# Ecogenomics/CheckM

Hardware: NVIDIA B200
Metric: genomes/hour (higher is better)
Workload: dtype int16 (SSV) / u8 (MSV) / int16 (Viterbi) / f32 (Forward, domain definition)

## Files before the change

### checkm_b200/csrc/device_utils.cuh

```cuda
#pragma once
#include <cuda_runtime.h>
#include <cstdint>

namespace ckm {

__device__ __forceinline__ uint32_t smem_u32(const void *p) { return (uint32_t)__cvta_generic_to_shared(p); }

__device__ __forceinline__ uint4 lds128(uint32_t addr) {
  uint4 v;
  asm volatile("ld.shared.v4.u32 {%0,%1,%2,%3}, [%4];" : "=r"(v.x), "=r"(v.y), "=r"(v.z), "=r"(v.w) : "r"(addr));
  return v;
}

__device__ __forceinline__ uint32_t prmt_b32(uint32_t a, uint32_t b, uint32_t c) {
  uint32_t d;
  asm("prmt.b32 %0, %1, %2, %3;" : "=r"(d) : "r"(a), "r"(b), "r"(c));
  return d;
}

__device__ __forceinline__ void mbar_init(uint64_t *bar, int count) {
  asm volatile("mbarrier.init.shared::cta.b64 [%0], %1;" ::"r"(smem_u32(bar)), "r"(count) : "memory");
}
__device__ __forceinline__ void fence_mbar_init() { asm volatile("fence.mbarrier_init.release.cluster;" ::: "memory"); }
__device__ __forceinline__ void fence_proxy_async() { asm volatile("fence.proxy.async.shared::cta;" ::: "memory"); }
__device__ __forceinline__ void mbar_expect_tx(uint64_t *bar, uint32_t bytes) {
  asm volatile("mbarrier.arrive.expect_tx.shared::cta.b64 _, [%0], %1;" ::"r"(smem_u32(bar)), "r"(bytes) : "memory");
}
__device__ __forceinline__ void bulk_g2s(uint32_t dst_smem, const void *src, uint32_t bytes, uint64_t *bar) {
  asm volatile("cp.async.bulk.shared::cluster.global.mbarrier::complete_tx::bytes [%0], [%1], %2, [%3];" ::"r"(dst_smem),
               "l"(src), "r"(bytes), "r"(smem_u32(bar))
               : "memory");
}
__device__ __forceinline__ void mbar_wait(uint64_t *bar, uint32_t parity) {
  asm volatile(
      "{\n"
      ".reg .pred p;\n"
      "WAIT_LOOP:\n"
      "mbarrier.try_wait.parity.shared::cta.b64 p, [%0], %1;\n"
      "@p bra WAIT_DONE;\n"
      "bra WAIT_LOOP;\n"
      "WAIT_DONE:\n"
      "}\n" ::"r"(smem_u32(bar)),
      "r"(parity)
      : "memory");
}

__device__ __forceinline__ int warp_max_int(int v) {
#pragma unroll
  for (int o = 16; o > 0; o >>= 1) v = max(v, __shfl_xor_sync(0xffffffffu, v, o));
  return v;
}
__device__ __forceinline__ float warp_sum_float(float v) {
#pragma unroll
  for (int o = 16; o > 0; o >>= 1) v += __shfl_xor_sync(0xffffffffu, v, o);
  return v;
}
__device__ __forceinline__ unsigned long long warp_sum_ull(unsigned long long v) {
#pragma unroll
  for (int o = 16; o > 0; o >>= 1) v += __shfl_xor_sync(0xffffffffu, v, o);
  return v;
}

__device__ __forceinline__ void atomicOr_u8(uint8_t *base, int64_t idx, unsigned bits) {
  unsigned *w = reinterpret_cast<unsigned *>(base + (idx & ~(int64_t)3));
  atomicOr(w, bits << (8 * (idx & 3)));
}

__device__ __forceinline__ double gumbel_surv(double x, double mu, double lambda) {
  const double y = lambda * (x - mu);
  const double ey = -exp(-y);
  if (fabs(ey) < 5e-9) return -ey;
  return 1.0 - exp(ey);
}
__device__ __forceinline__ double exp_surv(double x, double mu, double lambda) { return (x < mu) ? 1.0 : exp(-lambda * (x - mu)); }
__device__ __forceinline__ double exp_logsurv(double x, double mu, double lambda) { return (x < mu) ? 0.0 : -lambda * (x - mu); }

}
```

### checkm_b200/csrc/engine.hpp

```cpp
#pragma once
#include <cuda_runtime.h>
#include <cstdint>
#include <string>
#include <vector>
#include "../../include/ckm.h"
#include "hmm_model.hpp"

namespace ckm {
constexpr int MAX_MODEL_M = 4608;

constexpr int SSV_I8_WORDS = 8;
__host__ __device__ constexpr int ssv_row_bytes(int J) { return (J == 32) ? 128 * J - 16 * 32 * (SSV_I8_WORDS / 4 - 1) : 128 * J; }
__host__ __device__ constexpr int ssv_table_bytes(int J) { return KPAD * ssv_row_bytes(J); }
__host__ __device__ constexpr int ssv_block_bytes(int J) { return ssv_table_bytes(J) + 768; }
struct TileModel {
  int32_t model;
  int32_t slot0, nslots;
  int32_t chunk;
};

struct TileDesc {
  int32_t J;
  int32_t first_model;
  int32_t nmodels;
  int32_t chain_next;
  int32_t chain_prev;
  int32_t pad;
  int64_t table_off;
};

struct TileGroup {
  int32_t J;
  int32_t first_tile, ntiles;
  int32_t nchains;
  int32_t first_chain;
  int32_t pad;
  int64_t table_off;
  int64_t table_bytes;
};

struct ModelScalars {
  int32_t M;
  int32_t off_cells;
  int32_t Mpad;
  uint8_t tbm_b, tec_b, base_b, bias_b;
  int16_t base_w, xw_e_loop, xw_e_move;
  int16_t msv2_ok;
// ... 21 lines not shown
  EnvScratch, Envs1, EnvOrder1, Envs2, EnvOrder2,
  EnsRegions, EnsMultiIdx, EnsScratchOff, EnsScratch, EnsEnvs, EnsCount, EnsCaps, EnsEnvOff, EnsNeed,
  NtBytes, NtRows, NtPieces, NtStats, NtContigScaf, NtContigLen, NtCounters,
  Gather,
  Count
};

}

struct ckm_models {
  std::vector<ckm::Model> models;
  ckm::ModelScalars *d_scalars = nullptr;
  uint8_t  *d_rbv = nullptr;
  int16_t  *d_rwv = nullptr;
  int16_t  *d_twv = nullptr;
  float    *d_rfv = nullptr;
  float    *d_tfv = nullptr;
  float    *d_bias_eo = nullptr;
  uint4    *d_twb = nullptr;
  uint32_t *d_rmb = nullptr;
  uint32_t *d_rwb = nullptr;
  uint4    *d_twp = nullptr;
  uint32_t *d_rwp = nullptr;
  float4   *d_tfb = nullptr;
  float    *d_rfb = nullptr;
  int64_t   total_cols = 0;
  int       maxM = 0;
  std::vector<ckm::TileDesc>  tiles;
  std::vector<ckm::TileModel> tile_models;
  std::vector<ckm::TileGroup> groups;
  std::vector<int32_t>        chain_first_tile;
  std::vector<int32_t>        chain_ntiles;
  std::vector<int32_t>        ssv_bypass;
  int32_t        *d_ssv_bypass = nullptr;
  ckm::TileDesc  *d_tiles = nullptr;
  ckm::TileModel *d_tile_models = nullptr;
  ckm::TileGroup *d_groups = nullptr;
  int32_t        *d_chain_first_tile = nullptr, *d_chain_ntiles = nullptr;
  uint8_t        *d_tile_blob = nullptr;
  float          *d_tile_A = nullptr;
  int32_t        *d_tile_F = nullptr;
  int32_t        *d_tile_slot_model = nullptr;
  int64_t         tile_blob_bytes = 0;
  ckm_engine     *engine = nullptr;
};

struct ckm_seqdb {
  int32_t nseq = 0, nbins = 0;
  int64_t nres = 0;
  int64_t padded_bytes = 0;
  int32_t maxL = 0;
  std::vector<int64_t> offsets;
  std::vector<int32_t> bin_of_seq, bin_first_seq, bin_nseq;
  std::vector<int32_t> len;
  uint8_t *d_res = nullptr;
  int64_t *d_off = nullptr;
  int32_t *d_len = nullptr;
  int32_t *d_bin = nullptr;
  float   *d_nullsc = nullptr;
  int32_t *d_tjb = nullptr;
  float   *d_msvB = nullptr;
  float   *d_lenA = nullptr, *d_lenB = nullptr;
  int16_t *d_tmove_w = nullptr;
  int32_t *d_order = nullptr;
  int32_t *d_bin_nseq = nullptr;
  ckm_engine *engine = nullptr;
// ... 22 lines not shown
```

### checkm_b200/csrc/kernels_msv.cu

```cuda
#include <algorithm>
#include "engine.hpp"
#include "device_utils.cuh"
#include "stages.hpp"

namespace ckm {


template <int J> __host__ __device__ constexpr int tile_table_bytes() { return ssv_table_bytes(J); }
template <int J> __host__ __device__ constexpr int tile_block_bytes() { return ssv_block_bytes(J); }


template <int J>
__device__ __forceinline__ void ssv_rows(const uint8_t *__restrict__ res, int L, uint32_t tile_smem, int lane, uint32_t sel,
                                         const int16_t *bnd_in, int16_t *bnd_out, uint32_t (&u)[J], uint32_t &xE) {
  constexpr int G = J / 4;
  const uint4 *rp = reinterpret_cast<const uint4 *>(res);
  const uint32_t lane_off = tile_smem + lane * 16;
  constexpr bool I8 = (J == 32);
  constexpr int G0 = I8 ? SSV_I8_WORDS / 4 : 0;
  auto do_row = [&](uint32_t x, int i) {
    const uint32_t row = lane_off + x * ssv_row_bytes(J);
    uint4 e[G];
    if (I8) {
      const uint4 c = lds128(row);
      const uint32_t cw[4] = {c.x, c.y, c.z, c.w};
#pragma unroll
      for (int q = 0; q < SSV_I8_WORDS; ++q) (&e[q >> 2].x)[q & 3] = prmt_b32(cw[q >> 1], 0u, (q & 1) ? 0xB3A2u : 0x9180u);
    }
#pragma unroll
    for (int g = G0; g < G; ++g) e[g] = lds128(row + (g - (I8 ? G0 - 1 : 0)) * 512);
    uint32_t bndw = 0;
    if (bnd_in != nullptr) bndw = (i > 0) ? (uint32_t)(uint16_t)bnd_in[i - 1] : 0u;
    const uint32_t sh = __shfl_sync(0xffffffffu, u[J - 1], (lane + 31) & 31);
#pragma unroll
    for (int q = J - 1; q >= 1; --q) {
      const uint32_t d = (&e[q >> 2].x)[q & 3];
      u[q] = __viaddmax_s16x2_relu(u[q - 1], d, 0x80008000u);
    }
    const uint32_t p0 = __byte_perm(sh, bndw, sel);
    u[0] = __viaddmax_s16x2_relu(p0, e[0].x, 0x80008000u);
#pragma unroll
    for (int q = 0; q < J; q += 2) xE = __vimax3_s16x2(xE, u[q], u[q + 1]);
    if (bnd_out != nullptr && lane == 31) bnd_out[i] = (int16_t)(u[J - 1] >> 16);
  };
  const int nfull = L >> 4;
  uint4 cur = __ldg(rp);
  for (int b = 0; b < nfull; ++b) {
    const uint4 nxt = __ldg(rp + b + 1);
    const uint32_t w4[4] = {cur.x, cur.y, cur.z, cur.w};
#pragma unroll
    for (int r = 0; r < 16; ++r) do_row((w4[r >> 2] >> (8 * (r & 3))) & 0xffu, b * 16 + r);
    cur = nxt;
  }
  const int ntail = ((L & 15) + 3) >> 2;
  for (int t = 0; t < ntail; ++t) {
    const uint32_t w = (t == 0) ? cur.x : (t == 1) ? cur.y : (t == 2) ? cur.z : cur.w;
#pragma unroll
    for (int r = 0; r < 4; ++r) do_row((w >> (8 * r)) & 0xffu, nfull * 16 + t * 4 + r);
  }
}

template <int J>
__global__ void __launch_bounds__(SSV_WARPS * 32, 1) ssv_kernel(SsvParams p) {
  extern __shared__ __align__(128) uint8_t smem[];
  __shared__ __align__(8) uint64_t bar;
  __shared__ int s_unit, s_item;
  __shared__ int16_t su[SSV_WARPS][64];
  const int tid = threadIdx.x, lane = tid & 31, warp = tid >> 5;
  const uint32_t smem_base = smem_u32(smem);
  const uint32_t sel = (lane == 0) ? 0x1054u : 0x3210u;
  constexpr int TB = tile_block_bytes<J>();
  constexpr int I8CAP = (J == 32) ? 127 : 32767;
  if (tid == 0) { mbar_init(&bar, 1); fence_mbar_init(); }
  __syncthreads();
  uint32_t phase = 0;
  int cur_group = -1;
  unsigned long long my_cells = 0;
  int16_t *bndA = p.bnd ? p.bnd + ((int64_t)(blockIdx.x * SSV_WARPS + warp) * 2) * p.bnd_stride : nullptr;
  int16_t *bndB = p.bnd ? bndA + p.bnd_stride : nullptr;

  while (true) {
    __syncthreads();
    if (tid == 0) { s_unit = atomicAdd(p.unit_counter, 1); s_item = 0; }
    __syncthreads();
    const int unit = s_unit;
    if (unit >= p.ngroups * p.nchunks) break;
    const int gi = unit / p.nchunks, chunk = unit % p.nchunks;
    const TileGroup grp = p.groups[p.group_list[gi]];
    if (gi != cur_group) {
      cur_group = gi;
      if (tid == 0) {
        fence_proxy_async();
        mbar_expect_tx(&bar, (uint32_t)grp.table_bytes);
        for (int t = 0; t < grp.ntiles; ++t)
          bulk_g2s(smem_base + t * TB, p.tile_blob + grp.table_off + (int64_t)t * TB, TB, &bar);
      }
      mbar_wait(&bar, phase);
      phase ^= 1;
    }
    const int s_begin = chunk * p.seq_chunk;
    const int s_count = min(p.seq_chunk, p.nseq - s_begin);
    const int nitems = s_count * grp.nchains;
    while (true) {
      int it = 0;
      if (lane == 0) it = atomicAdd(&s_item, 1);
      it = __shfl_sync(0xffffffffu, it, 0);
      if (it >= nitems) break;
      const int s = p.order[s_begin + it / grp.nchains];
      const int chain = grp.first_chain + it % grp.nchains;
      const int L = p.len[s];
      if (L == 0) continue;
      const int t0 = p.chain_first_tile[chain], nt = p.chain_ntiles[chain];
      const int sbin = p.bin[s];
      if (p.tile_active != nullptr && !p.tile_active[(int64_t)sbin * p.ntiles + t0]) continue;
      const uint8_t *res = p.res + p.off[s];
      const float Bs = p.msvB[s];
      const int tjb = p.tjb[s];
      bool chain_cand = false;
      for (int tt = 0; tt < nt; ++tt) {
        const int t = t0 + tt;
        const int tl = t - grp.first_tile;
        const uint32_t tsm = smem_base + tl * TB;
        uint32_t u[J];
#pragma unroll
        for (int q = 0; q < J; ++q) u[q] = 0u;
        uint32_t xE = 0u;
        const int16_t *bin_ = (nt > 1 && tt > 0) ? ((tt & 1) ? bndA : bndB) : nullptr;
        int16_t *bout = (nt > 1 && tt + 1 < nt) ? ((tt & 1) ? bndB : bndA) : nullptr;
        ssv_rows<J>(res, L, tsm, lane, sel, bin_, bout, u, xE);
        my_cells += (unsigned long long)L * (2 * J);
        const uint8_t *meta = smem + tl * TB + tile_table_bytes<J>();
        const float *A = reinterpret_cast<const float *>(meta);
        const int32_t *F = reinterpret_cast<const int32_t *>(meta + 256);
        const int32_t *SM = reinterpret_cast<const int32_t *>(meta + 512);
        const int ulo = (int)(int16_t)(xE & 0xffffu), uhi = (int)(int16_t)(xE >> 16);
        const int thr_lo = min(min((int)floorf(A[lane] + Bs) - 1, F[lane] + tjb), I8CAP);
        const int thr_hi = min(min((int)floorf(A[32 + lane] + Bs) - 1, F[32 + lane] + tjb), I8CAP);
        const bool c_lo = (SM[lane] >= 0) && (ulo >= thr_lo);
        const bool c_hi = (SM[32 + lane] >= 0) && (uhi >= thr_hi);
        const unsigned m_lo = __ballot_sync(0xffffffffu, c_lo), m_hi = __ballot_sync(0xffffffffu, c_hi);
        if ((m_lo | m_hi) == 0u) continue;
        if (nt > 1) { chain_cand = true; continue; }
        su[warp][lane] = (int16_t)ulo; su[warp][32 + lane] = (int16_t)uhi;
        __syncwarp();
        const TileDesc td = p.tiles[t];
        if (lane < td.nmodels) {
          const TileModel tm = p.tile_models[td.first_model + lane];
          const unsigned long long mask = ((unsigned long long)m_hi << 32) | m_lo;
          const unsigned long long range = ((tm.nslots >= 64) ? ~0ull : ((1ull << tm.nslots) - 1ull)) << tm.slot0;
          bool act = (mask & range) != 0ull;
          if (act && p.model_active != nullptr) act = p.model_active[(int64_t)sbin * p.nmodels + tm.model] != 0;
          if (act) {
            int umax = 0;
            for (int z = tm.slot0; z < tm.slot0 + tm.nslots; ++z) umax = max(umax, (int)su[warp][z]);
            const int jbound = min(F[tm.slot0] + tjb, I8CAP);
            if (!p.resolve || umax >= jbound || umax < 1) {
              const int pos = atomicAdd(p.cand_count, 1);
              if (pos < p.cand_cap) p.cand[pos] = make_int2(s, tm.model);
            } else {
              const ModelScalars ms = p.ms[tm.model];
              const int tjbm = min(tjb + (int)ms.tbm_b, 255);
              const int xB0 = max((int)ms.base_b - tjbm, 0);
              const int xJ = max(umax + xB0 - (int)ms.tec_b, 0);
              float usc = ((float)(xJ - tjb) - (float)ms.base_b);
              usc = __fdiv_rn(usc, ms.scale_b);
              usc = __fsub_rn(usc, 3.0f);
              if (p.xj_dense != nullptr) p.xj_dense[(int64_t)p.model_slot[tm.model] * p.nseq + s] = xJ;
              const float nullsc = p.nullsc[s];
              const float seq_score = __fdiv_rn(__fsub_rn(usc, nullsc), 0.69314718055994529f);
              const double P = gumbel_surv((double)seq_score, (double)ms.evparam[0], (double)ms.evparam[1]);
              atomicAdd(p.resolved_count, 1);
              if (P <= p.F1) {
                const int pos = atomicAdd(p.pass_count, 1);
                if (pos < p.pass_cap) {
                  Candidate cd;
                  cd.seq = s; cd.model = tm.model; cd.usc = usc; cd.filtersc = nullsc; cd.vitsc = 0.f; cd.fwdsc = 0.f; cd.P = P;
                  p.pass[pos] = cd;
                }
              }
            }
          }
        }
        __syncwarp();
      }
      if (nt > 1 && chain_cand && lane == 0) {
        const TileModel tm = p.tile_models[p.tiles[t0].first_model];
        bool act = true;
        if (p.model_active != nullptr) act = p.model_active[(int64_t)sbin * p.nmodels + tm.model] != 0;
        if (act) {
          const int pos = atomicAdd(p.cand_count, 1);
          if (pos < p.cand_cap) p.cand[pos] = make_int2(s, tm.model);
        }
      }
    }
  }
  my_cells = warp_sum_ull(my_cells);
  if (lane == 0 && p.cells != nullptr) atomicAdd(p.cells, my_cells);
}

template __global__ void ssv_kernel<4>(SsvParams);
template __global__ void ssv_kernel<8>(SsvParams);
template __global__ void ssv_kernel<16>(SsvParams);
template __global__ void ssv_kernel<32>(SsvParams);

int launch_ssv(int J, const SsvParams &p, int grid, size_t smem_bytes, cudaStream_t stream) {
  cudaError_t e;
  switch (J) {
    case 4:
      e = cudaFuncSetAttribute(ssv_kernel<4>, cudaFuncAttributeMaxDynamicSharedMemorySize, (int)smem_bytes);
      if (e != cudaSuccess) return cuda_fail(e, "cudaFuncSetAttribute(ssv<4>)");
      ssv_kernel<4><<<grid, SSV_WARPS * 32, smem_bytes, stream>>>(p);
      break;
    case 8:
      e = cudaFuncSetAttribute(ssv_kernel<8>, cudaFuncAttributeMaxDynamicSharedMemorySize, (int)smem_bytes);
      if (e != cudaSuccess) return cuda_fail(e, "cudaFuncSetAttribute(ssv<8>)");
      ssv_kernel<8><<<grid, SSV_WARPS * 32, smem_bytes, stream>>>(p);
      break;
    case 16:
      e = cudaFuncSetAttribute(ssv_kernel<16>, cudaFuncAttributeMaxDynamicSharedMemorySize, (int)smem_bytes);
      if (e != cudaSuccess) return cuda_fail(e, "cudaFuncSetAttribute(ssv<16>)");
      ssv_kernel<16><<<grid, SSV_WARPS * 32, smem_bytes, stream>>>(p);
      break;
    case 32:
      e = cudaFuncSetAttribute(ssv_kernel<32>, cudaFuncAttributeMaxDynamicSharedMemorySize, (int)smem_bytes);
      if (e != cudaSuccess) return cuda_fail(e, "cudaFuncSetAttribute(ssv<32>)");
      ssv_kernel<32><<<grid, SSV_WARPS * 32, smem_bytes, stream>>>(p);
      break;
    default: set_error("unsupported tile width"); return CKM_EINVAL;
  }
  e = cudaGetLastError();
  if (e != cudaSuccess) return cuda_fail(e, "ssv_kernel launch");
  return CKM_OK;
}



__global__ void __launch_bounds__(MSV_WARPS * 32) msv_exact_kernel(MsvParams p) {
  extern __shared__ __align__(128) uint8_t smem[];
  const int lane = threadIdx.x & 31, warp = threadIdx.x >> 5;
  uint8_t *row0 = smem + (size_t)warp * 2 * p.row_bytes, *row1 = row0 + p.row_bytes;
  const int ncand = min(*p.cand_count, p.cand_cap);
  for (int c = blockIdx.x * MSV_WARPS + warp; c < ncand; c += gridDim.x * MSV_WARPS) {
    const int2 pr = p.cand[c];
    const int s = pr.x, m = pr.y;
    const ModelScalars ms = p.ms[m];
    if (p.use_blk && ms.msv2_ok) continue;
    const int M = ms.M, L = p.len[s];
    const uint8_t *res = p.res + p.off[s];
    const uint8_t *rbv = p.rbv + (int64_t)ms.off_cells * KPAD;
    const int tjb = p.tjb[s];
    const int tjbm = min(tjb + (int)ms.tbm_b, 255);
    const int bias = ms.bias_b, base = ms.base_b, tec = ms.tec_b;
    for (int k = lane; k <= M + 1; k += 32) { row0[k] = 0; row1[k] = 0; }
    __syncwarp();
    int xJ = 0, xB = max(base - tjbm, 0);
    bool overflow = false;
    uint8_t *prev = row0, *cur = row1;
    for (int i = 0; i < L; ++i) {
      const int x = res[i];
      const uint8_t *rsc = rbv + (int64_t)x * ms.Mpad;
      int xE = 0;
      for (int k = lane + 1; k <= M; k += 32) {
        int sv = max((int)prev[k - 1], xB);
        sv = min(sv + bias, 255);
        sv = max(sv - (int)rsc[k], 0);
// ... 235 lines not shown
```

### checkm_b200/csrc/models.cu

```cuda
#include <algorithm>
#include <cmath>
#include <cstdlib>
#include <cstring>
#include <fstream>
#include <stdexcept>
#include "engine.hpp"

namespace ckm {

static thread_local std::string g_error;
void set_error(const std::string &msg) { g_error = msg; }
const std::string &get_error() { return g_error; }
int cuda_fail(cudaError_t e, const char *what) {
  set_error(std::string("CUDA error: ") + cudaGetErrorString(e) + " in " + what);
  return CKM_ECUDA;
}

static const double kLog2 = 0.69314718055994529;

template <class T>
static int upload(T **dptr, const std::vector<T> &h) {
  size_t bytes = std::max<size_t>(h.size() * sizeof(T), 16);
  CKM_CUDA(cudaMalloc((void **)dptr, bytes));
  if (!h.empty()) CKM_CUDA(cudaMemcpy(*dptr, h.data(), h.size() * sizeof(T), cudaMemcpyHostToDevice));
  return CKM_OK;
}

static int tile_block_bytes_host(int J) { return ssv_block_bytes(J); }

static void build_tiles(ckm_models &db, std::vector<uint8_t> &blob) {
  const int n = (int)db.models.size();
  struct Item { int model, M; };
  const char *pol = std::getenv("CKM_SSV_J");
  int fixedJ = 32;
  if (pol != nullptr) { if (!std::strcmp(pol, "auto")) fixedJ = 0; else fixedJ = std::atoi(pol); }
  if (fixedJ != 0 && fixedJ != 4 && fixedJ != 8 && fixedJ != 16 && fixedJ != 32) fixedJ = 32;
  std::vector<Item> cls[3], longm;
  int Js[3] = {4, 8, 16};
  int chainJ = 16;
  if (fixedJ != 0) { Js[0] = Js[1] = Js[2] = fixedJ; chainJ = (fixedJ == 32) ? 16 : fixedJ; }
  for (int i = 0; i < n; ++i) {
    int M = db.models[i].M;
    if (fixedJ != 0) { if (M <= 64 * fixedJ - 1) cls[0].push_back({i, M}); else longm.push_back({i, M}); }
    else if (M <= 255) cls[0].push_back({i, M});
    else if (M <= 511) cls[1].push_back({i, M});
    else if (M <= 1023) cls[2].push_back({i, M});
    else longm.push_back({i, M});
  }
  struct HostTile { int J; std::vector<TileModel> tm; int used; int chain_prev, chain_next; };
  std::vector<HostTile> tiles;
  std::vector<std::pair<int, int>> chains;
  std::vector<int> tile_class;
  for (int c = 0; c < 3; ++c) {
    auto &v = cls[c];
    std::stable_sort(v.begin(), v.end(), [](const Item &a, const Item &b) { return a.M > b.M; });
    const int J = Js[c];
    size_t first = tiles.size();
    for (const Item &it : v) {
      int W = it.M / J + 1;
      size_t t;
      for (t = first; t < tiles.size(); ++t)
        if (tiles[t].used + W <= 64 && (int)tiles[t].tm.size() < 32) break;
      if (t == tiles.size()) { tiles.push_back({J, {}, 0, 0, 0}); tile_class.push_back(c); }
      tiles[t].tm.push_back({it.model, tiles[t].used, W, 0});
      tiles[t].used += W;
    }
    for (size_t t = first; t < tiles.size(); ++t) chains.push_back({(int)t, 1});
  }
  const int chunk_cells = 64 * chainJ;
  const int64_t cap = 200000;
  db.ssv_bypass.clear();
  for (const Item &it : longm) {
    int ncells = it.M + 1;
    int nch = (ncells + chunk_cells - 1) / chunk_cells;
    if ((int64_t)nch * tile_block_bytes_host(chainJ) > cap) { db.ssv_bypass.push_back(it.model); continue; }
    chains.push_back({(int)tiles.size(), nch});
    for (int c = 0; c < nch; ++c) {
      HostTile ht{chainJ, {}, 64, c > 0, c + 1 < nch};
      ht.tm.push_back({it.model, 0, 64, c});
      tiles.push_back(ht);
      tile_class.push_back(3);
    }
  }
  db.tiles.clear(); db.tile_models.clear(); db.groups.clear(); db.chain_first_tile.clear(); db.chain_ntiles.clear();
  int64_t off = 0;
  for (size_t t = 0; t < tiles.size(); ++t) {
    TileDesc td{};
    td.J = tiles[t].J; td.first_model = (int)db.tile_models.size(); td.nmodels = (int)tiles[t].tm.size();
    td.chain_next = tiles[t].chain_next; td.chain_prev = tiles[t].chain_prev; td.table_off = off;
    for (auto &tm : tiles[t].tm) db.tile_models.push_back(tm);
    db.tiles.push_back(td);
    off += tile_block_bytes_host(td.J);
  }
  blob.assign((size_t)off, 0);
  {
    TileGroup g{}; bool open = false; int64_t gbytes = 0;
    for (size_t c = 0; c < chains.size(); ++c) {
      int t0 = chains[c].first, nt = chains[c].second, J = tiles[t0].J;
      int64_t need = (int64_t)nt * tile_block_bytes_host(J);
      if (need > cap) throw std::runtime_error("model " + db.models[tiles[t0].tm[0].model].name + " is too long for the SSV tiles");
      if (open && (g.J != J || gbytes + need > cap)) { g.table_bytes = gbytes; db.groups.push_back(g); open = false; }
      if (!open) { g = TileGroup{}; g.J = J; g.first_tile = t0; g.ntiles = 0; g.nchains = 0; g.first_chain = (int)c; g.table_off = db.tiles[t0].table_off; gbytes = 0; open = true; }
      g.ntiles += nt; g.nchains += 1; gbytes += need;
      db.chain_first_tile.push_back(t0); db.chain_ntiles.push_back(nt);
    }
    if (open) { g.table_bytes = gbytes; db.groups.push_back(g); }
  }
  for (size_t t = 0; t < tiles.size(); ++t) {
    const int J = tiles[t].J;
    uint8_t *base = blob.data() + db.tiles[t].table_off;
    const bool i8 = (J == 32);
    const int RB = ssv_row_bytes(J);
    float *A = reinterpret_cast<float *>(base + ssv_table_bytes(J));
    int32_t *F = reinterpret_cast<int32_t *>(base + ssv_table_bytes(J) + 256);
    int32_t *SM = reinterpret_cast<int32_t *>(base + ssv_table_bytes(J) + 512);
    for (int s = 0; s < 64; ++s) { A[s] = 1e30f; F[s] = 1 << 28; SM[s] = -1; }
    auto put = [&](int x, int lane, int half, int q, int d) {
      uint8_t *row = base + (size_t)x * RB;
      if (i8 && q < SSV_I8_WORDS) reinterpret_cast<int8_t *>(row)[lane * 16 + 2 * q + half] = (int8_t)std::max(d, -128);
      else {
        const int g = (q >> 2) - (i8 ? (SSV_I8_WORDS / 4 - 1) : 0);
        reinterpret_cast<int16_t *>(row + ((size_t)g * 32 + lane) * 16)[(q & 3) * 2 + half] = (int16_t)std::max(d, -32768);
      }
    };
    for (int x = 0; x < KPAD; ++x) for (int lane = 0; lane < 32; ++lane) for (int half = 0; half < 2; ++half) for (int q = 0; q < J; ++q) put(x, lane, half, q, -32768);
    for (size_t j = 0; j < tiles[t].tm.size(); ++j) {
      const TileModel &tm = tiles[t].tm[j];
      const Model &m = db.models[tm.model];
      const int W1 = m.M + 1;
      for (int sl = 0; sl < tm.nslots; ++sl) {
        const int slot = tm.slot0 + sl;
        A[slot] = db.models[tm.model].M > 0 ? 0.0f : 0.0f;
        SM[slot] = (int)j;
        const int lane = slot & 31, half = slot >> 5;
        for (int q = 0; q < J; ++q) {
          const int k = tm.chunk * 64 * J + sl * J + q + 1;
          if (k > m.M) continue;
          for (int x = 0; x < KP; ++x) {
            put(x, lane, half, q, (int)m.bias_b - (int)m.rbv[(size_t)x * W1 + k]);
          }
        }
      }
    }
  }
  for (size_t t = 0; t < tiles.size(); ++t) {
    const int J = tiles[t].J;
    uint8_t *base = blob.data() + db.tiles[t].table_off;
    float *A = reinterpret_cast<float *>(base + ssv_table_bytes(J));
    int32_t *F = reinterpret_cast<int32_t *>(base + ssv_table_bytes(J) + 256);
    for (auto &tm : tiles[t].tm) {
      const Model &m = db.models[tm.model];
      const double F1 = 0.02;
      const double sstar = (double)m.evparam[0] - std::log(-std::log(1.0 - F1)) / (double)m.evparam[1];
      const float Am = (float)((double)m.tbm_b + (double)m.tec_b + (double)m.scale_b * kLog2 * sstar);
      for (int sl = 0; sl < tm.nslots; ++sl) { A[tm.slot0 + sl] = Am; F[tm.slot0 + sl] = 4 + (int)m.tbm_b; }
    }
  }
}

int models_build_device(ckm_models &db) {
  const int n = (int)db.models.size();
  std::vector<ModelScalars> sc(n);
  int64_t cols = 0, blk_units = 0;
  db.maxM = 0;
  for (int i = 0; i < n; ++i) {
    const Model &m = db.models[i];
    ModelScalars &s = sc[i];
    std::memset(&s, 0, sizeof(s));
    s.M = m.M; s.Mpad = ((m.M + 1) + 31) / 32 * 32 + 32; s.off_cells = (int32_t)cols;
    cols += s.Mpad;
    s.tbm_b = m.tbm_b; s.tec_b = m.tec_b; s.base_b = m.base_b; s.bias_b = m.bias_b;
    s.base_w = m.base_w; s.xw_e_loop = m.xw_e_loop; s.xw_e_move = m.xw_e_move;
    s.scale_b = m.scale_b; s.scale_w = m.scale_w;
    for (int z = 0; z < 6; ++z) s.evparam[z] = m.evparam[z];
    s.ddbound_w = m.ddbound_w;
    {
      int emax = 0, tbm = 0;
      for (int x = 0; x < KP; ++x) for (int k = 1; k <= m.M; ++k) emax = std::max(emax, (int)m.rwv[(size_t)x * (m.M + 1) + k]);
      for (int k = 1; k <= m.M; ++k) tbm = std::min(tbm, (int)m.twv[(size_t)k * T_N + 0]);
      s.vit_emax = (int16_t)emax; s.vit_tbm = (int16_t)tbm;
    }
    s.vq = (m.M <= 64) ? 2 : (m.M <= 128) ? 4 : (m.M <= 192) ? 6 : (m.M <= 256) ? 8 : (m.M <= 384) ? 12 : (m.M <= 512) ? 16 : (m.M <= 640) ? 20 : (m.M <= 768) ? 24 : (m.M <= 896) ? 28 : (m.M <= 1024) ? 32 : 0;
// ... 127 lines not shown
```

### checkm_b200/csrc/search.cu

```cuda
#include <algorithm>
#include <atomic>
#include <chrono>
#include <cstdio>
#include <cmath>
#include <cstdlib>
#include <cstring>
#include <vector>
#include "engine.hpp"
#include "stages.hpp"
#include "pool.hpp"

using namespace ckm;

namespace ckm {

std::atomic<int> g_live_engines{0};

static bool use_blocked_kernels();
static bool use_packed_viterbi() { const char *v = std::getenv("CKM_VITP"); return use_blocked_kernels() && !(v != nullptr && v[0] == '0'); }
static int fan_out(ckm_engine *e);
static int fan_in(ckm_engine *e);
enum { CTR_UNIT4 = 0, CTR_UNIT8, CTR_UNIT16, CTR_UNIT32, CTR_CAND, CTR_MSV, CTR_BIAS, CTR_VIT, CTR_FWD, CTR_ENV, CTR_DOM, CTR_VREDO, CTR_SSVRES, CTR_VWORK = 16 , CTR_N = 32 };

struct ActiveMasks {
// ... 86 lines not shown
  if (!flat.empty()) CKM_CUDA(cudaMemcpyAsync(glist, flat.data(), sizeof(int32_t) * flat.size(), cudaMemcpyHostToDevice, st));
  CKM_CUDA(cudaStreamSynchronize(st));

  CKM_CUDA(cudaEventRecord(e->ev[0], st));
  const int Js[4] = {4, 8, 16, 32};
  for (int c = 0; c < 4; ++c) {
    if (gl[c].empty() || db->nseq == 0) continue;
    SsvParams p{};
    p.res = db->d_res; p.off = db->d_off; p.len = db->d_len; p.bin = db->d_bin;
    p.msvB = db->d_msvB; p.tjb = db->d_tjb; p.order = db->d_order;
    p.nseq = db->nseq;
    p.seq_chunk = 128;
    p.nchunks = (db->nseq + p.seq_chunk - 1) / p.seq_chunk;
    p.groups = m->d_groups; p.group_list = glist + goff[c]; p.ngroups = (int32_t)gl[c].size();
    p.tiles = m->d_tiles; p.tile_models = m->d_tile_models;
    p.chain_first_tile = m->d_chain_first_tile; p.chain_ntiles = m->d_chain_ntiles;
    p.tile_blob = m->d_tile_blob;
    p.tile_active = am.tile_active; p.model_active = am.model_active;
    p.ntiles = (int32_t)m->tiles.size(); p.nmodels = (int32_t)m->models.size();
    p.unit_counter = e->d_counters + CTR_UNIT4 + c;
    p.cand = s1.cand; p.cand_count = e->d_counters + CTR_CAND; p.cand_cap = s1.cand_cap;
    p.bnd = bnd; p.bnd_stride = bnd_stride;
    p.cells = s1.cells;
    { const char *v = std::getenv("CKM_SSV_RESOLVE"); p.resolve = (v != nullptr && v[0] == '0') ? 0 : 1; }
    p.ms = m->d_scalars; p.nullsc = db->d_nullsc;
    p.pass = s1.pass; p.pass_count = e->d_counters + CTR_MSV; p.pass_cap = s1.pass_cap;
    p.resolved_count = e->d_counters + CTR_SSVRES;
    p.xj_dense = xj_dense; p.model_slot = am.model_slot;
    p.F1 = 0.02;
    int64_t maxbytes = 0;
    for (int g : gl[c]) maxbytes = std::max<int64_t>(maxbytes, m->groups[g].table_bytes);
    const int64_t units = (int64_t)p.ngroups * p.nchunks;
    const int grid = (int)std::min<int64_t>(nsm, units);
    if ((rc = launch_ssv(Js[c], p, grid, (size_t)maxbytes, st))) return rc;
    e->stats.kernel_launches++;
  }
  if (!m->ssv_bypass.empty()) {
    if ((rc = launch_ssv_bypass(m->d_ssv_bypass, (int32_t)m->ssv_bypass.size(), db->nseq, db->d_len, db->d_bin,
                                am.model_active, (int32_t)m->models.size(), s1.cand, e->d_counters + CTR_CAND, s1.cand_cap, st))) return rc;
    e->stats.kernel_launches++;
  }
  CKM_CUDA(cudaEventRecord(e->ev[1], st));
  {
    MsvParams p{};
    p.res = db->d_res; p.off = db->d_off; p.len = db->d_len; p.nullsc = db->d_nullsc; p.tjb = db->d_tjb;
    p.ms = m->d_scalars; p.rbv = m->d_rbv; p.rmb = m->d_rmb;
    p.cand = s1.cand; p.cand_count = e->d_counters + CTR_CAND; p.cand_cap = s1.cand_cap;
    p.out = s1.pass; p.out_count = e->d_counters + CTR_MSV; p.out_cap = s1.pass_cap;
    p.xj_dense = xj_dense; p.model_slot = am.model_slot; p.nseq = db->nseq;
    p.row_bytes = (m->maxM + 2 + 15) / 16 * 16;
    p.F1 = 0.02;
    p.use_blk = use_blocked_kernels() ? 1 : 0;
    if ((rc = fan_out(e))) return rc;
    if (p.use_blk) { for (int c = 0; c < N_BLK_CLASSES; ++c) if ((rc = launch_msv2(p, c, nsm * 16, e->cls[c]))) return rc; }
    if ((rc = launch_msv_exact(p, nsm * 4, e->cls[N_BLK_CLASSES]))) return rc;
    if ((rc = fan_in(e))) return rc;
    e->stats.kernel_launches += 1 + (p.use_blk ? N_BLK_CLASSES : 0);
  }
  CKM_CUDA(cudaEventRecord(e->ev[2], st));
  return CKM_OK;
}


struct Stage2 {
  Candidate *a = nullptr, *b = nullptr, *redo = nullptr;
  int32_t cap = 0;
  Candidate *fwd_list = nullptr;
// ... 722 lines not shown
```

### checkm_b200/csrc/stages.hpp

```cpp
#pragma once
#include "engine.hpp"

namespace ckm {

#ifndef CKM_SSV_WARPS
#define CKM_SSV_WARPS 16
#endif
constexpr int SSV_WARPS = CKM_SSV_WARPS;
constexpr int SSV_WARPS_HOST = SSV_WARPS;
constexpr int MSV_WARPS = 8;

struct SsvParams {
  const uint8_t *res; const int64_t *off; const int32_t *len; const int32_t *bin;
  const float *msvB; const int32_t *tjb; const int32_t *order;
  int32_t nseq, seq_chunk, nchunks;
  const TileGroup *groups; const int32_t *group_list; int32_t ngroups;
  const TileDesc *tiles; const TileModel *tile_models;
  const int32_t *chain_first_tile, *chain_ntiles;
  const uint8_t *tile_blob;
  const uint8_t *tile_active;
  const uint8_t *model_active;
  int32_t ntiles, nmodels;
  int32_t *unit_counter;
  int2 *cand; int32_t *cand_count; int32_t cand_cap;
  int16_t *bnd; int64_t bnd_stride;
  unsigned long long *cells;
  int32_t resolve;
  const ModelScalars *ms; const float *nullsc;
  Candidate *pass; int32_t *pass_count; int32_t pass_cap;
  int32_t *resolved_count;
  int32_t *xj_dense; const int32_t *model_slot;
  double F1;
};

int launch_ssv(int J, const SsvParams &p, int grid, size_t smem_bytes, cudaStream_t stream);

struct MsvParams {
  const uint8_t *res; const int64_t *off; const int32_t *len;
  const float *nullsc; const int32_t *tjb;
  const ModelScalars *ms; const uint8_t *rbv; const uint32_t *rmb;
  const int2 *cand; const int32_t *cand_count; int32_t cand_cap;
  Candidate *out; int32_t *out_count; int32_t out_cap;
  int32_t *xj_dense;
  const int32_t *model_slot;
  int32_t nseq;
  int32_t row_bytes;
  int32_t use_blk;
  double F1;
};

int launch_msv_exact(const MsvParams &p, int grid, cudaStream_t stream);
int launch_ssv_bypass(const int32_t *models, int32_t nbypass, int32_t nseq, const int32_t *len, const int32_t *bin,
                      const uint8_t *model_active, int32_t nmodels_db, int2 *cand, int32_t *cand_count, int32_t cand_cap,
                      cudaStream_t stream);
int launch_msv2(const MsvParams &p, int cls, int grid, cudaStream_t stream);

constexpr int VIT_WARPS = 4;
constexpr int FWD_WARPS = 4;
struct FilterParams {
  const uint8_t *res; const int64_t *off; const int32_t *len;
  const float *lenA, *lenB;
  const int16_t *tmove_w;
  const ModelScalars *ms;
  const float *bias_eo; const int16_t *rwv; const int16_t *twv; const float *rfv; const float *tfv;
  const uint4 *twb; const uint32_t *rwb; const float4 *tfb; const float *rfb;
  const uint4 *twp; const uint32_t *rwp;
  Candidate *redo; int32_t *redo_count; int32_t redo_cap;
  int32_t *vit_work;
// ... 60 lines not shown
```

Measured before the change: 40590.

## Stage part of J=32 SSV emission tables in tensor memory instead of int8 chunk

For J=32 SSV tiles, the first sixteen words of each emission row are copied from shared memory into TMEM after the bulk load, and read back with tcgen05.ld during the recurrence in place of the previous int8-compressed chunk. This aims to cut shared-memory load pressure in the inner loop and drop the int8 saturation cap. In exchange, each CTA allocates all 512 TMEM columns and adds fences and a copy pass per group. Each J=32 chain is also forced into its own group with a single tile, which changes grouping and chaining for long models and may change results or performance for multi-tile chains.

```diff
diff --git a/checkm_b200/csrc/device_utils.cuh b/checkm_b200/csrc/device_utils.cuh
--- a/checkm_b200/csrc/device_utils.cuh
+++ b/checkm_b200/csrc/device_utils.cuh
@@ -45,6 +45,34 @@
       : "memory");
 }
 
+__device__ __forceinline__ void tmem_alloc(uint32_t *dst_smem, uint32_t ncols) {
+  asm volatile("tcgen05.alloc.cta_group::1.sync.aligned.shared::cta.b32 [%0], %1;" ::"r"(smem_u32(dst_smem)), "r"(ncols) : "memory");
+}
+__device__ __forceinline__ void tmem_release(uint32_t taddr, uint32_t ncols) {
+  asm volatile("tcgen05.relinquish_alloc_permit.cta_group::1.sync.aligned;" ::: "memory");
+  asm volatile("tcgen05.dealloc.cta_group::1.sync.aligned.b32 %0, %1;" ::"r"(taddr), "r"(ncols) : "memory");
+}
+__device__ __forceinline__ void tmem_fence_before_sync() { asm volatile("tcgen05.fence::before_thread_sync;" ::: "memory"); }
+__device__ __forceinline__ void tmem_fence_after_sync() { asm volatile("tcgen05.fence::after_thread_sync;" ::: "memory"); }
+__device__ __forceinline__ void tmem_ld16(uint32_t taddr, uint32_t (&r)[16]) {
+  asm volatile("tcgen05.ld.sync.aligned.32x32b.x16.b32 {%0,%1,%2,%3,%4,%5,%6,%7,%8,%9,%10,%11,%12,%13,%14,%15}, [%16];"
+               : "=r"(r[0]), "=r"(r[1]), "=r"(r[2]), "=r"(r[3]), "=r"(r[4]), "=r"(r[5]), "=r"(r[6]), "=r"(r[7]),
+                 "=r"(r[8]), "=r"(r[9]), "=r"(r[10]), "=r"(r[11]), "=r"(r[12]), "=r"(r[13]), "=r"(r[14]), "=r"(r[15])
+               : "r"(taddr));
+}
+__device__ __forceinline__ void tmem_wait_ld(uint32_t (&r)[16]) {
+  asm volatile("tcgen05.wait::ld.sync.aligned;" ::: "memory");
+#pragma unroll
+  for (int j = 0; j < 16; ++j) asm volatile("" : "+r"(r[j]));
+}
+__device__ __forceinline__ void tmem_st16(uint32_t taddr, const uint32_t (&r)[16]) {
+  asm volatile("tcgen05.st.sync.aligned.32x32b.x16.b32 [%0], {%1,%2,%3,%4,%5,%6,%7,%8,%9,%10,%11,%12,%13,%14,%15,%16};"
+               ::"r"(taddr), "r"(r[0]), "r"(r[1]), "r"(r[2]), "r"(r[3]), "r"(r[4]), "r"(r[5]), "r"(r[6]), "r"(r[7]),
+                 "r"(r[8]), "r"(r[9]), "r"(r[10]), "r"(r[11]), "r"(r[12]), "r"(r[13]), "r"(r[14]), "r"(r[15])
+               : "memory");
+}
+__device__ __forceinline__ void tmem_wait_st() { asm volatile("tcgen05.wait::st.sync.aligned;" ::: "memory"); }
+
 __device__ __forceinline__ int warp_max_int(int v) {
 #pragma unroll
   for (int o = 16; o > 0; o >>= 1) v = max(v, __shfl_xor_sync(0xffffffffu, v, o));
diff --git a/checkm_b200/csrc/engine.hpp b/checkm_b200/csrc/engine.hpp
--- a/checkm_b200/csrc/engine.hpp
+++ b/checkm_b200/csrc/engine.hpp
@@ -10,9 +10,14 @@
 constexpr int MAX_MODEL_M = 4608;
 
 constexpr int SSV_I8_WORDS = 8;
-__host__ __device__ constexpr int ssv_row_bytes(int J) { return (J == 32) ? 128 * J - 16 * 32 * (SSV_I8_WORDS / 4 - 1) : 128 * J; }
-__host__ __device__ constexpr int ssv_table_bytes(int J) { return KPAD * ssv_row_bytes(J); }
-__host__ __device__ constexpr int ssv_block_bytes(int J) { return ssv_table_bytes(J) + 768; }
+constexpr int SSV_TMEM_WORDS = 16;
+static_assert(KPAD * SSV_TMEM_WORDS <= 512, "a TMEM-assisted tile must fit the 512 tensor-memory columns of an SM");
+__host__ __device__ constexpr bool ssv_int8_chunk(int J, bool tmem) { return J == 32 && !tmem; }
+__host__ __device__ constexpr int ssv_row_bytes(int J, bool tmem) {
+  return ssv_int8_chunk(J, tmem) ? 128 * J - 16 * 32 * (SSV_I8_WORDS / 4 - 1) : 128 * J;
+}
+__host__ __device__ constexpr int ssv_table_bytes(int J, bool tmem) { return KPAD * ssv_row_bytes(J, tmem); }
+__host__ __device__ constexpr int ssv_block_bytes(int J, bool tmem) { return ssv_table_bytes(J, tmem) + 768; }
 struct TileModel {
   int32_t model;
   int32_t slot0, nslots;
@@ -100,6 +105,7 @@
   std::vector<int32_t>        chain_first_tile;
   std::vector<int32_t>        chain_ntiles;
   std::vector<int32_t>        ssv_bypass;
+  bool            ssv_tmem = true;
   int32_t        *d_ssv_bypass = nullptr;
   ckm::TileDesc  *d_tiles = nullptr;
   ckm::TileModel *d_tile_models = nullptr;
diff --git a/checkm_b200/csrc/kernels_msv.cu b/checkm_b200/csrc/kernels_msv.cu
--- a/checkm_b200/csrc/kernels_msv.cu
+++ b/checkm_b200/csrc/kernels_msv.cu
@@ -6,21 +6,24 @@
 namespace ckm {
 
 
-template <int J> __host__ __device__ constexpr int tile_table_bytes() { return ssv_table_bytes(J); }
-template <int J> __host__ __device__ constexpr int tile_block_bytes() { return ssv_block_bytes(J); }
-
-
-template <int J>
-__device__ __forceinline__ void ssv_rows(const uint8_t *__restrict__ res, int L, uint32_t tile_smem, int lane, uint32_t sel,
-                                         const int16_t *bnd_in, int16_t *bnd_out, uint32_t (&u)[J], uint32_t &xE) {
+template <int J, bool TM> __host__ __device__ constexpr int tile_table_bytes() { return ssv_table_bytes(J, TM); }
+template <int J, bool TM> __host__ __device__ constexpr int tile_block_bytes() { return ssv_block_bytes(J, TM); }
+constexpr uint32_t SSV_TMEM_COLS = 512;
+
+template <int J, bool TM>
+__device__ __forceinline__ void ssv_rows(const uint8_t *__restrict__ res, int L, uint32_t tile_smem, uint32_t tmem_lane, int lane,
+                                         uint32_t sel, const int16_t *bnd_in, int16_t *bnd_out, uint32_t (&u)[J], uint32_t &xE) {
   constexpr int G = J / 4;
   const uint4 *rp = reinterpret_cast<const uint4 *>(res);
   const uint32_t lane_off = tile_smem + lane * 16;
-  constexpr bool I8 = (J == 32);
-  constexpr int G0 = I8 ? SSV_I8_WORDS / 4 : 0;
+  constexpr bool I8 = ssv_int8_chunk(J, TM);
+  constexpr int G0 = I8 ? SSV_I8_WORDS / 4 : TM ? SSV_TMEM_WORDS / 4 : 0;
+  static_assert(!TM || J == 32, "TMEM-assisted tiles are J = 32 tiles");
   auto do_row = [&](uint32_t x, int i) {
-    const uint32_t row = lane_off + x * ssv_row_bytes(J);
+    const uint32_t row = lane_off + x * ssv_row_bytes(J, TM);
     uint4 e[G];
+    uint32_t t[TM ? SSV_TMEM_WORDS : 1];
+    if constexpr (TM) tmem_ld16(tmem_lane + x * SSV_TMEM_WORDS, t);
     if (I8) {
       const uint4 c = lds128(row);
       const uint32_t cw[4] = {c.x, c.y, c.z, c.w};
@@ -29,6 +32,11 @@
     }
 #pragma unroll
     for (int g = G0; g < G; ++g) e[g] = lds128(row + (g - (I8 ? G0 - 1 : 0)) * 512);
+    if constexpr (TM) {
+      tmem_wait_ld(t);
+#pragma unroll
+      for (int q = 0; q < SSV_TMEM_WORDS; ++q) (&e[q >> 2].x)[q & 3] = t[q];
+    }
     uint32_t bndw = 0;
     if (bnd_in != nullptr) bndw = (i > 0) ? (uint32_t)(uint16_t)bnd_in[i - 1] : 0u;
     const uint32_t sh = __shfl_sync(0xffffffffu, u[J - 1], (lane + 31) & 31);
@@ -60,19 +68,27 @@
   }
 }
 
-template <int J>
+template <int J, bool TM>
 __global__ void __launch_bounds__(SSV_WARPS * 32, 1) ssv_kernel(SsvParams p) {
+  static_assert(!TM || SSV_WARPS % 4 == 0, "every sub-partition needs warps to fill its copy of the TMEM words");
   extern __shared__ __align__(128) uint8_t smem[];
   __shared__ __align__(8) uint64_t bar;
   __shared__ int s_unit, s_item;
+  __shared__ uint32_t s_tmem;
   __shared__ int16_t su[SSV_WARPS][64];
   const int tid = threadIdx.x, lane = tid & 31, warp = tid >> 5;
   const uint32_t smem_base = smem_u32(smem);
   const uint32_t sel = (lane == 0) ? 0x1054u : 0x3210u;
-  constexpr int TB = tile_block_bytes<J>();
-  constexpr int I8CAP = (J == 32) ? 127 : 32767;
-  if (tid == 0) { mbar_init(&bar, 1); fence_mbar_init(); }
+  constexpr int TB = tile_block_bytes<J, TM>();
+  constexpr int I8CAP = ssv_int8_chunk(J, TM) ? 127 : 32767;
+  if (warp == 0) {
+    if (TM) tmem_alloc(&s_tmem, SSV_TMEM_COLS);
+    if (lane == 0) { mbar_init(&bar, 1); fence_mbar_init(); }
+  }
+  if (TM) tmem_fence_before_sync();
   __syncthreads();
+  if (TM) tmem_fence_after_sync();
+  const uint32_t tmem_lane = TM ? s_tmem + ((uint32_t)(32 * (warp & 3)) << 16) : 0u;
   uint32_t phase = 0;
   int cur_group = -1;
   unsigned long long my_cells = 0;
@@ -80,7 +96,9 @@
   int16_t *bndB = p.bnd ? bndA + p.bnd_stride : nullptr;
 
   while (true) {
+    if (TM) tmem_fence_before_sync();
     __syncthreads();
+    if (TM) tmem_fence_after_sync();
     if (tid == 0) { s_unit = atomicAdd(p.unit_counter, 1); s_item = 0; }
     __syncthreads();
     const int unit = s_unit;
@@ -97,6 +115,22 @@
       }
       mbar_wait(&bar, phase);
       phase ^= 1;
+      if constexpr (TM) {
+        for (int x = warp >> 2; x < KPAD; x += SSV_WARPS / 4) {
+          const uint32_t row = smem_base + lane * 16 + x * ssv_row_bytes(J, TM);
+          uint32_t w[SSV_TMEM_WORDS];
+#pragma unroll
+          for (int g = 0; g < SSV_TMEM_WORDS / 4; ++g) {
+            const uint4 v = lds128(row + g * 512);
+            w[4 * g] = v.x; w[4 * g + 1] = v.y; w[4 * g + 2] = v.z; w[4 * g + 3] = v.w;
+          }
+          tmem_st16(tmem_lane + x * SSV_TMEM_WORDS, w);
+        }
+        tmem_wait_st();
+        tmem_fence_before_sync();
+        __syncthreads();
+        tmem_fence_after_sync();
+      }
     }
     const int s_begin = chunk * p.seq_chunk;
     const int s_count = min(p.seq_chunk, p.nseq - s_begin);
@@ -110,7 +144,7 @@
       const int chain = grp.first_chain + it % grp.nchains;
       const int L = p.len[s];
       if (L == 0) continue;
-      const int t0 = p.chain_first_tile[chain], nt = p.chain_ntiles[chain];
+      const int t0 = p.chain_first_tile[chain], nt = TM ? 1 : p.chain_ntiles[chain];
       const int sbin = p.bin[s];
       if (p.tile_active != nullptr && !p.tile_active[(int64_t)sbin * p.ntiles + t0]) continue;
       const uint8_t *res = p.res + p.off[s];
@@ -127,9 +161,9 @@
         uint32_t xE = 0u;
         const int16_t *bin_ = (nt > 1 && tt > 0) ? ((tt & 1) ? bndA : bndB) : nullptr;
         int16_t *bout = (nt > 1 && tt + 1 < nt) ? ((tt & 1) ? bndB : bndA) : nullptr;
-        ssv_rows<J>(res, L, tsm, lane, sel, bin_, bout, u, xE);
+        ssv_rows<J, TM>(res, L, tsm, tmem_lane, lane, sel, bin_, bout, u, xE);
         my_cells += (unsigned long long)L * (2 * J);
-        const uint8_t *meta = smem + tl * TB + tile_table_bytes<J>();
+        const uint8_t *meta = smem + tl * TB + tile_table_bytes<J, TM>();
         const float *A = reinterpret_cast<const float *>(meta);
         const int32_t *F = reinterpret_cast<const int32_t *>(meta + 256);
         const int32_t *SM = reinterpret_cast<const int32_t *>(meta + 512);
@@ -194,43 +228,35 @@
       }
     }
   }
+  if (TM && warp == 0) tmem_release(s_tmem, SSV_TMEM_COLS);
   my_cells = warp_sum_ull(my_cells);
   if (lane == 0 && p.cells != nullptr) atomicAdd(p.cells, my_cells);
 }
 
-template __global__ void ssv_kernel<4>(SsvParams);
-template __global__ void ssv_kernel<8>(SsvParams);
-template __global__ void ssv_kernel<16>(SsvParams);
-template __global__ void ssv_kernel<32>(SsvParams);
-
-int launch_ssv(int J, const SsvParams &p, int grid, size_t smem_bytes, cudaStream_t stream) {
-  cudaError_t e;
-  switch (J) {
-    case 4:
-      e = cudaFuncSetAttribute(ssv_kernel<4>, cudaFuncAttributeMaxDynamicSharedMemorySize, (int)smem_bytes);
-      if (e != cudaSuccess) return cuda_fail(e, "cudaFuncSetAttribute(ssv<4>)");
-      ssv_kernel<4><<<grid, SSV_WARPS * 32, smem_bytes, stream>>>(p);
-      break;
-    case 8:
-      e = cudaFuncSetAttribute(ssv_kernel<8>, cudaFuncAttributeMaxDynamicSharedMemorySize, (int)smem_bytes);
-      if (e != cudaSuccess) return cuda_fail(e, "cudaFuncSetAttribute(ssv<8>)");
-      ssv_kernel<8><<<grid, SSV_WARPS * 32, smem_bytes, stream>>>(p);
-      break;
-    case 16:
-      e = cudaFuncSetAttribute(ssv_kernel<16>, cudaFuncAttributeMaxDynamicSharedMemorySize, (int)smem_bytes);
-      if (e != cudaSuccess) return cuda_fail(e, "cudaFuncSetAttribute(ssv<16>)");
-      ssv_kernel<16><<<grid, SSV_WARPS * 32, smem_bytes, stream>>>(p);
-      break;
-    case 32:
-      e = cudaFuncSetAttribute(ssv_kernel<32>, cudaFuncAttributeMaxDynamicSharedMemorySize, (int)smem_bytes);
-      if (e != cudaSuccess) return cuda_fail(e, "cudaFuncSetAttribute(ssv<32>)");
-      ssv_kernel<32><<<grid, SSV_WARPS * 32, smem_bytes, stream>>>(p);
-      break;
-    default: set_error("unsupported tile width"); return CKM_EINVAL;
-  }
+template __global__ void ssv_kernel<4, false>(SsvParams);
+template __global__ void ssv_kernel<8, false>(SsvParams);
+template __global__ void ssv_kernel<16, false>(SsvParams);
+template __global__ void ssv_kernel<32, false>(SsvParams);
+template __global__ void ssv_kernel<32, true>(SsvParams);
+
+template <int J, bool TM>
+static int launch_ssv_t(const SsvParams &p, int grid, size_t smem_bytes, cudaStream_t stream) {
+  cudaError_t e = cudaFuncSetAttribute(ssv_kernel<J, TM>, cudaFuncAttributeMaxDynamicSharedMemorySize, (int)smem_bytes);
+  if (e != cudaSuccess) return cuda_fail(e, "cudaFuncSetAttribute(ssv_kernel)");
+  ssv_kernel<J, TM><<<grid, SSV_WARPS * 32, smem_bytes, stream>>>(p);
   e = cudaGetLastError();
   if (e != cudaSuccess) return cuda_fail(e, "ssv_kernel launch");
   return CKM_OK;
+}
+
+int launch_ssv(int J, bool tmem, const SsvParams &p, int grid, size_t smem_bytes, cudaStream_t stream) {
+  switch (J) {
+    case 4: return launch_ssv_t<4, false>(p, grid, smem_bytes, stream);
+    case 8: return launch_ssv_t<8, false>(p, grid, smem_bytes, stream);
+    case 16: return launch_ssv_t<16, false>(p, grid, smem_bytes, stream);
+    case 32: return tmem ? launch_ssv_t<32, true>(p, grid, smem_bytes, stream) : launch_ssv_t<32, false>(p, grid, smem_bytes, stream);
+    default: set_error("unsupported tile width"); return CKM_EINVAL;
+  }
 }
 
 
diff --git a/checkm_b200/csrc/models.cu b/checkm_b200/csrc/models.cu
--- a/checkm_b200/csrc/models.cu
+++ b/checkm_b200/csrc/models.cu
@@ -26,8 +26,6 @@
   return CKM_OK;
 }
 
-static int tile_block_bytes_host(int J) { return ssv_block_bytes(J); }
-
 static void build_tiles(ckm_models &db, std::vector<uint8_t> &blob) {
   const int n = (int)db.models.size();
   struct Item { int model, M; };
@@ -35,6 +33,8 @@
   int fixedJ = 32;
   if (pol != nullptr) { if (!std::strcmp(pol, "auto")) fixedJ = 0; else fixedJ = std::atoi(pol); }
   if (fixedJ != 0 && fixedJ != 4 && fixedJ != 8 && fixedJ != 16 && fixedJ != 32) fixedJ = 32;
+  { const char *v = std::getenv("CKM_SSV_TMEM"); db.ssv_tmem = !(v != nullptr && v[0] == '0'); }
+  const bool tmem = db.ssv_tmem;
   std::vector<Item> cls[3], longm;
   int Js[3] = {4, 8, 16};
   int chainJ = 16;
@@ -73,7 +73,7 @@
   for (const Item &it : longm) {
     int ncells = it.M + 1;
     int nch = (ncells + chunk_cells - 1) / chunk_cells;
-    if ((int64_t)nch * tile_block_bytes_host(chainJ) > cap) { db.ssv_bypass.push_back(it.model); continue; }
+    if ((int64_t)nch * ssv_block_bytes(chainJ, tmem) > cap) { db.ssv_bypass.push_back(it.model); continue; }
     chains.push_back({(int)tiles.size(), nch});
     for (int c = 0; c < nch; ++c) {
       HostTile ht{chainJ, {}, 64, c > 0, c + 1 < nch};
@@ -90,16 +90,16 @@
     td.chain_next = tiles[t].chain_next; td.chain_prev = tiles[t].chain_prev; td.table_off = off;
     for (auto &tm : tiles[t].tm) db.tile_models.push_back(tm);
     db.tiles.push_back(td);
-    off += tile_block_bytes_host(td.J);
+    off += ssv_block_bytes(td.J, tmem);
   }
   blob.assign((size_t)off, 0);
   {
     TileGroup g{}; bool open = false; int64_t gbytes = 0;
     for (size_t c = 0; c < chains.size(); ++c) {
       int t0 = chains[c].first, nt = chains[c].second, J = tiles[t0].J;
-      int64_t need = (int64_t)nt * tile_block_bytes_host(J);
+      int64_t need = (int64_t)nt * ssv_block_bytes(J, tmem);
       if (need > cap) throw std::runtime_error("model " + db.models[tiles[t0].tm[0].model].name + " is too long for the SSV tiles");
-      if (open && (g.J != J || gbytes + need > cap)) { g.table_bytes = gbytes; db.groups.push_back(g); open = false; }
+      if (open && (g.J != J || gbytes + need > cap || (tmem && J == 32))) { g.table_bytes = gbytes; db.groups.push_back(g); open = false; }
       if (!open) { g = TileGroup{}; g.J = J; g.first_tile = t0; g.ntiles = 0; g.nchains = 0; g.first_chain = (int)c; g.table_off = db.tiles[t0].table_off; gbytes = 0; open = true; }
       g.ntiles += nt; g.nchains += 1; gbytes += need;
       db.chain_first_tile.push_back(t0); db.chain_ntiles.push_back(nt);
@@ -109,11 +109,11 @@
   for (size_t t = 0; t < tiles.size(); ++t) {
     const int J = tiles[t].J;
     uint8_t *base = blob.data() + db.tiles[t].table_off;
-    const bool i8 = (J == 32);
-    const int RB = ssv_row_bytes(J);
-    float *A = reinterpret_cast<float *>(base + ssv_table_bytes(J));
-    int32_t *F = reinterpret_cast<int32_t *>(base + ssv_table_bytes(J) + 256);
-    int32_t *SM = reinterpret_cast<int32_t *>(base + ssv_table_bytes(J) + 512);
+    const bool i8 = ssv_int8_chunk(J, tmem);
+    const int RB = ssv_row_bytes(J, tmem);
+    float *A = reinterpret_cast<float *>(base + ssv_table_bytes(J, tmem));
+    int32_t *F = reinterpret_cast<int32_t *>(base + ssv_table_bytes(J, tmem) + 256);
+    int32_t *SM = reinterpret_cast<int32_t *>(base + ssv_table_bytes(J, tmem) + 512);
     for (int s = 0; s < 64; ++s) { A[s] = 1e30f; F[s] = 1 << 28; SM[s] = -1; }
     auto put = [&](int x, int lane, int half, int q, int d) {
       uint8_t *row = base + (size_t)x * RB;
@@ -146,8 +146,8 @@
   for (size_t t = 0; t < tiles.size(); ++t) {
     const int J = tiles[t].J;
     uint8_t *base = blob.data() + db.tiles[t].table_off;
-    float *A = reinterpret_cast<float *>(base + ssv_table_bytes(J));
-    int32_t *F = reinterpret_cast<int32_t *>(base + ssv_table_bytes(J) + 256);
+    float *A = reinterpret_cast<float *>(base + ssv_table_bytes(J, tmem));
+    int32_t *F = reinterpret_cast<int32_t *>(base + ssv_table_bytes(J, tmem) + 256);
     for (auto &tm : tiles[t].tm) {
       const Model &m = db.models[tm.model];
       const double F1 = 0.02;
diff --git a/checkm_b200/csrc/search.cu b/checkm_b200/csrc/search.cu
--- a/checkm_b200/csrc/search.cu
+++ b/checkm_b200/csrc/search.cu
@@ -142,7 +142,7 @@
     for (int g : gl[c]) maxbytes = std::max<int64_t>(maxbytes, m->groups[g].table_bytes);
     const int64_t units = (int64_t)p.ngroups * p.nchunks;
     const int grid = (int)std::min<int64_t>(nsm, units);
-    if ((rc = launch_ssv(Js[c], p, grid, (size_t)maxbytes, st))) return rc;
+    if ((rc = launch_ssv(Js[c], m->ssv_tmem, p, grid, (size_t)maxbytes, st))) return rc;
     e->stats.kernel_launches++;
   }
   if (!m->ssv_bypass.empty()) {
diff --git a/checkm_b200/csrc/stages.hpp b/checkm_b200/csrc/stages.hpp
--- a/checkm_b200/csrc/stages.hpp
+++ b/checkm_b200/csrc/stages.hpp
@@ -33,7 +33,7 @@
   double F1;
 };
 
-int launch_ssv(int J, const SsvParams &p, int grid, size_t smem_bytes, cudaStream_t stream);
+int launch_ssv(int J, bool tmem, const SsvParams &p, int grid, size_t smem_bytes, cudaStream_t stream);
 
 struct MsvParams {
   const uint8_t *res; const int64_t *off; const int32_t *len;
```

Result: faster. 45270 (median of 6 runs) (+11.5%).
